# forestagostinelli/DeepCubeA

Hardware: AMD Instinct MI355X
Metric: A* nodes expanded/sec on cube3, batch 20k (higher is better)
Workload: dtype u8 states / f64 cost keys / f32 heuristic

## Files before the change

### deepcubea_amd/csrc/dca_engine.hip

```cpp
#include <string.h>

#include <new>
#include <vector>

#include "dca_common.h"
#include "dca_tile.h"

namespace dca {

constexpr int NBIN = 4096;
constexpr int kBinsPerThread = NBIN / 1024;
constexpr int kLgNbin = 12;
constexpr int kSub = 2048;
constexpr int kScanBlocks = 256;
constexpr int kCollectBlocks = 512;
constexpr int kRankBlocks = 256;
constexpr uint32_t kTinyBin = 512;
constexpr int kSortCap = 8192;
constexpr int RT = 512;
constexpr int kRegEnt = 16;
constexpr uint32_t kLdsEnt = RT * kRegEnt;
constexpr int kStash = 2560;
constexpr int kSegs = NBIN + 1 + kSub;
constexpr uint32_t kGiantBin = 8192;
constexpr int kMaxLevels = 9;
constexpr unsigned long long kBarrierTimeout = 200000000ull;
constexpr unsigned long long kBarrierTimeoutFirst = 25000000ull;
constexpr uint32_t GBAR_BROKEN = 0x80000000u;
constexpr uint32_t NIL = 0xFFFFFFFFu;
constexpr uint32_t ID_MASK = 0x7FFFFFFFu, ID_SOLVED = 0x80000000u;
constexpr uint64_t EMPTY = ~0ull;
constexpr uint64_t DEAD = ~0ull;
constexpr uint32_t GINF = 0xFFFFFFFFu;
constexpr int kMaxMoves = 4096;

struct Slot {
    uint64_t entry;
    uint32_t g;
    uint32_t head;
};

struct alignas(128) Cnt {
    uint32_t v;
    uint32_t pad[31];
};
struct alignas(128) GRange {
    uint64_t kmin, kmax;
    uint32_t imin, imax;
    uint32_t pad[26];
};
struct alignas(128) Rng {
    uint64_t kmin, kmax;
    uint64_t pad[14];
};
struct IterState {
    uint32_t pool_n;
    uint32_t npop, m, base;
    uint32_t best_id;
    int32_t has_best;
    float best_cost;
};
struct Ctl {
    int32_t done, failed, stop_after, pad0;
    int64_t iters, gen, expanded;
    IterState S[2];
    uint32_t cur_f;
    uint32_t hbin;
    uint32_t front_above;
    uint32_t cur_b;
    uint64_t T;
    uint32_t refill, compact, r_bstar, spill_bin, r_move;
    uint64_t r_kmin;
    uint32_t r_shift;
    uint32_t want, bstar, shift, n_big, n_ord;
    uint32_t giant;
    uint32_t tseg;
    uint32_t pre_b, cn_star;
    uint64_t sel_kmin;
    uint32_t goal_id;
    uint32_t dbg_nord, dbg_maxbin, dbg_giant, dbg_giant_seen, dbg_maxsub;
    Cnt open_n[4];
    Cnt closed_n, back_dead, front_dead, ret_n, ticket_a;
    Cnt gbar;
    GRange grange;
    Rng rng[4];
    alignas(128) unsigned long long goal_best;
    alignas(128) uint32_t first_solved;
};

__device__ __forceinline__ uint64_t key_of_cost(double c) {
    uint64_t b = (uint64_t)__double_as_longlong(c);
    return (b & 0x8000000000000000ull) ? ~b : (b | 0x8000000000000000ull);
}
__device__ __forceinline__ double cost_of_key(uint64_t k) {
    uint64_t b = (k & 0x8000000000000000ull) ? (k & 0x7FFFFFFFFFFFFFFFull) : ~k;
    return __longlong_as_double((long long)b);
}
__device__ __forceinline__ uint32_t select_shift(uint64_t kmin, uint64_t kmax) {
    uint64_t range = kmax - kmin;
    int bits = range ? 64 - __clzll((long long)range) : 0;
    return bits > kLgNbin ? (uint32_t)(bits - kLgNbin) : 0u;
}
__device__ __forceinline__ uint32_t bin_of(uint64_t k, uint64_t kmin, uint32_t shift) {
    if (k <= kmin) return 0u;
    const uint64_t f = (k - kmin) >> shift;
    return f < (uint64_t)NBIN ? (uint32_t)f : (uint32_t)(NBIN - 1);
}
__device__ __forceinline__ bool pair_less(uint64_t ka, uint32_t ia, uint64_t kb, uint32_t ib) {
    return ka < kb || (ka == kb && (ia & ID_MASK) < (ib & ID_MASK));
}

enum {
    P_REFILL_HIST = 0, P_REFILL_SCAN, P_REFILL_MOVE, P_SEL_HIST, P_SEL_SCAN, P_SEL_COLLECT, P_RANK, P_EXPAND,
    P_PROBE,
    P_DECIDE, P_PACK, P_COMMIT, P_RANK_SMALL, P_RANK_BIG, P_RB_LOAD, P_RB_COUNT, P_RB_SCATTER, P_RB_ORDER, P_COUNT
};
constexpr int kProfSlots = 1024;
__device__ int g_back_squeeze_mark;
__device__ int g_first_barrier_gives_up;
__device__ __forceinline__ uint32_t rank_shares(uint32_t cn) {
    return cn <= (uint32_t)(512 * 16) ? (cn + 1023u) / 1024u : 1u;
}

struct Eng {
    int env, dim, D, A, B, sem, oh_dtype, depth;
    double w;
    float wf;
    uint32_t max_nodes, M, tab_cap, tab_mask;
    uint32_t front_cap;
    uint8_t* state;
    int32_t* g;
    uint32_t* parent;
    uint8_t* move;
    uint8_t* solved;
    Slot* tab;
    uint32_t* closed_slots;
    uint64_t* open_key[4];
    uint32_t* open_id[4];
    uint32_t f_keep, f_max;
    uint32_t *hist, *pre, *fill;
    uint32_t* rhist;
    uint32_t* subhist;
    int coop;
    uint32_t* coop_off;
    uint64_t* part;
    uint64_t* tmp_key;
    uint32_t* tmp_id;
    uint16_t* tmp_f;
    uint32_t* tmp_idx;
    uint64_t* ord_key;
    uint32_t* ord_id;
    uint32_t* big_list;
    uint64_t* pop_key;
    uint32_t *pop_id, *pop_g;
// ... 660 lines not shown
        s_nbig = 0;
        s_spill = NBIN;
        s_bstar = 0;
        s_hbin = NBIN;
    }
    scan_vals(hv, pre, wsum);
    const uint32_t n = rebased ? (cb ? on1 : on0) : (cb ? on1 : on0) - dead0 - above0;
    const uint32_t want = n < (uint32_t)E.B ? n : (uint32_t)E.B;
    const uint32_t hwant = (uint32_t)(kRefillPeriod + 2) * (uint32_t)E.B;
    for (int k = 0; k < kBinsPerThread; k++) {
        int bin = kBinsPerThread * t + k;
        if (pre[bin] < want && want <= pre[bin + 1]) s_bstar = (uint32_t)bin;
        if (rebased && n > E.f_max) {
            const uint32_t keepn = want + front_keep(E);
            if (pre[bin] < keepn && keepn <= pre[bin + 1]) s_spill = (uint32_t)bin;
        }
        if (rebased && pre[bin] < hwant && hwant <= pre[bin + 1]) s_hbin = (uint32_t)bin + 1u;
        E.pre[bin] = pre[bin];
        E.fill[bin] = 0;
    }
    for (int i = NBIN + t; i < kSegs; i += 1024) E.fill[i] = 0;
    if (t == 1023) E.pre[NBIN] = pre[NBIN];
    __syncthreads();
    const bool giant = E.coop && !*E.coop_off && want != 0 && pre[s_bstar + 1] - pre[s_bstar] > kGiantBin;
    if (giant)
        for (int i = t; i < kMaxLevels * kSub; i += 1024) E.subhist[i] = 0;
    for (int k = 0; k < kBinsPerThread; k++) {
        const uint32_t bin = kBinsPerThread * t + k;
        if (bin <= s_bstar && want != 0) {
            const uint32_t cn = pre[bin + 1] - pre[bin];
            if (cn > 256) atomicMax(&s_maxbin, cn);
            if (cn > (uint32_t)kSortCap) atomicAdd(&s_giant, 1u);
            if (cn > kTinyBin && !(giant && bin == s_bstar)) {
                uint32_t G = rank_shares(cn);
                G = G > 8u ? 8u : G;
                const uint32_t at = atomicAdd(&s_nbig, G);
                for (uint32_t g = 0; g < G; g++) E.big_list[at + g] = bin | (g << 16) | (G << 20);
            }
        }
    }
    __syncthreads();
    if (t == 0) {
        if (rebased) {
            uint64_t fmn = ~0ull, fmx = 0;
            for (int w = 0; w < 16; w++) {
                fmn = s_red[0][w] < fmn ? s_red[0][w] : fmn;
                fmx = s_red[1][w] > fmx ? s_red[1][w] : fmx;
            }
            c->cur_f = cb;
            c->rng[cb].kmin = fmn;
            c->rng[cb].kmax = fmx;
            c->hbin = s_hbin;
        }
        if (refill) {
            if (compact) {
                c->cur_b ^= 1;
                c->back_dead.v = 0;
                c->compact = 0;
            }
            c->refill = 0;
        }
        c->want = want;
        c->bstar = s_bstar;
        c->tseg = s_bstar;
        c->pre_b = pre[s_bstar];
        c->cn_star = pre[s_bstar + 1] - pre[s_bstar];
        c->giant = giant ? 1u : 0u;
        c->gbar.v = 0;
        c->grange.kmin = ~0ull;
        c->grange.kmax = 0;
// ... 259 lines not shown
            subpre[PER * t + k] = run;
            if (run < need && need <= run + v[k]) L.tsub = PER * t + k;
            run += v[k];
        }
        if (t == 255) subpre[kSub] = run;
        __syncthreads();
        tsub = L.tsub;
        if (tsub == ~0u) {
            if (t == 0) c->failed = 1, c->done = 1;
            return BAR_FAIL;
        }
        const uint32_t cn = subpre[tsub + 1] - subpre[tsub];
        if (cn <= kGiantBin || shc == 0 || lvl + 1 >= kMaxLevels) break;
        below += subpre[tsub];
        need -= subpre[tsub];
        V0 += (u128)tsub << shc;
        span = ((u128)1 << shc) - 1;
        __syncthreads();
    }
    const uint32_t seg0 = bstar + 1u;
    if (blockIdx.x == 0) {
        if (t == 0) {
            L.nb = c->n_big;
            E.pre[bstar + 1] = pre_b + below;
            c->tseg = seg0 + tsub;
            c->n_ord = pre_b + below + subpre[tsub + 1];
            c->dbg_nord = pre_b + below + subpre[tsub + 1];
        }
        __syncthreads();
        for (uint32_t sg = t; sg <= tsub + 1u; sg += 256) {
            const uint32_t cn = sg == 0 ? below : subpre[sg] - subpre[sg - 1];
            if (sg > 0) E.pre[seg0 + sg] = pre_b + below + subpre[sg];
            if (cn > kTinyBin) {
                uint32_t G = rank_shares(cn);
                G = G > 8u ? 8u : G;
                const uint32_t at = atomicAdd(&L.nb, G);
                for (uint32_t g = 0; g < G; g++) E.big_list[at + g] = (bstar + sg) | (g << 16) | (G << 20);
            }
        }
        __syncthreads();
        if (t == 0) c->n_big = L.nb;
    }
    uint32_t* lcnt = L.lcnt;
    for (uint32_t i = t; i < (uint32_t)(kSegs + 3); i += 256) lcnt[i] = 0;
    if (t == 0) {
        L.st_n = 0;
        L.nz_n = 0;
    }
    __syncthreads();
    uint64_t* st_key = L.u.g.st_key;
    uint32_t* st_idx = L.u.g.st_idx;
    uint16_t *st_f = L.u.g.st_f, *nzf = L.u.g.nzf;
    auto seg_base = [&](uint32_t f) -> uint32_t {
        return f < bstar ? L.pre[f] : f == bstar ? pre_b : pre_b + below + subpre[f - seg0];
    };
    auto seg_end = [&](uint32_t f) -> uint32_t {
        return f < bstar ? L.pre[f + 1] : f == bstar ? pre_b + below : pre_b + below + subpre[f - seg0 + 1];
    };
    auto flush = [&]() {
        const uint32_t ns = L.st_n < (uint32_t)kStashG ? L.st_n : (uint32_t)kStashG;
        const uint32_t nz = L.nz_n;
        for (uint32_t i = t; i < nz; i += 256) {
            const uint32_t f = nzf[i];
            lcnt[f] = atomicAdd(&E.fill[f], lcnt[f]);
        }
        __syncthreads();
        for (uint32_t p = t; p < ns; p += 256) {
            const uint32_t f = st_f[p];
            const uint32_t id = ids[st_idx[p]];
            const uint32_t pos = seg_base(f) + atomicAdd(&lcnt[f], 1u);
// ... 122 lines not shown
        const uint32_t want = P.want;
#pragma unroll
        for (int k = 0; k < PER; k++) {
            L.pre[PER * t + k] = run;
            if (run < want && want <= run + v[k]) L.bstar = PER * t + k;
            run += v[k];
        }
        if (t == 255) L.pre[NBIN] = run;
        __syncthreads();
        if (want == 0) {
            if (blockIdx.x == 0 && t == 0) {
                c->failed = 1;
                c->done = 1;
            }
            return;
        }
        P.bstar = L.bstar;
        P.pre_b = L.pre[P.bstar];
        P.cn_star = L.pre[P.bstar + 1] - P.pre_b;
        P.giant = E.coop && !*E.coop_off && P.cn_star > kGiantBin;
        if (blockIdx.x == 0) {
            for (uint32_t i = t; i <= (uint32_t)NBIN; i += 256) E.pre[i] = L.pre[i];
            if (t == 0) {
                L.nb = 0;
                L.st_n = 0;
                L.nz_n = 0;
            }
            __syncthreads();
            for (uint32_t bin = t; bin <= P.bstar; bin += 256) {
                const uint32_t cn = L.pre[bin + 1] - L.pre[bin];
                if (cn > 256) atomicMax(&L.st_n, cn);
                if (cn > (uint32_t)kSortCap) atomicAdd(&L.nz_n, 1u);
                if (cn > kTinyBin && !(P.giant && bin == P.bstar)) {
                    uint32_t G = rank_shares(cn);
                    G = G > 8u ? 8u : G;
                    const uint32_t at = atomicAdd(&L.nb, G);
                    for (uint32_t g = 0; g < G; g++) E.big_list[at + g] = bin | (g << 16) | (G << 20);
                }
            }
            __syncthreads();
            if (t == 0) {
                c->bstar = P.bstar;
                c->tseg = P.bstar;
                c->giant = P.giant ? 1u : 0u;
                c->pre_b = P.pre_b;
                c->cn_star = P.cn_star;
                c->spill_bin = NBIN;
                c->n_big = L.nb;
                c->n_ord = L.pre[P.bstar + 1];
                c->front_dead.v += want;
                c->dbg_nord = L.pre[P.bstar + 1];
                c->dbg_maxbin = L.st_n;
                c->dbg_giant = L.nz_n;
                c->dbg_giant_seen += L.nz_n;
                c->dbg_maxsub = 0;
            }
            __syncthreads();
        }
    } else {
        P.bstar = c->bstar;
        P.giant = c->giant != 0;
        P.pre_b = c->pre_b;
        P.cn_star = c->cn_star;
        if (P.want == 0) return;
        for (uint32_t i = t; i <= P.bstar + 1u; i += 256) L.pre[i] = E.pre[i];
        __syncthreads();
    }
    if (P.giant) {
        if (collect_giant(E, c, L, P) != BAR_BROKEN) return;
        if (blockIdx.x == 0 && t == 0) {
            const uint32_t cn = P.cn_star;
            uint32_t G = rank_shares(cn);
            G = G > 8u ? 8u : G;
            const uint32_t at = c->n_big;
            if (cn > kTinyBin) {
                for (uint32_t g = 0; g < G; g++) E.big_list[at + g] = P.bstar | (g << 16) | (G << 20);
                c->n_big = at + G;
            }
            c->giant = 0;
        }
        P.giant = false;
        __syncthreads();
    }
    const uint32_t n = P.n;
    const uint64_t kmin = P.kmin;
    const uint32_t shift = P.shift, bstar = P.bstar;
    uint64_t* __restrict__ keys = E.open_key[P.b];
    const uint32_t* __restrict__ ids = E.open_id[P.b];
    constexpr uint32_t ITEMS = 8, TILE = 256 * ITEMS;
    const uint32_t ntiles = (n + TILE - 1) / TILE;
    uint64_t* st_key = L.u.n.st_key;
    uint32_t* st_idx = L.u.n.st_idx;
    uint16_t *st_f = L.u.n.st_f, *nzf = L.u.n.nzf;
    for (int i = t; i < NBIN; i += 256) L.lcnt[i] = 0;
    if (t == 0) {
        L.st_n = 0;
        L.nz_n = 0;
    }
    __syncthreads();
    auto flush = [&]() {
        const uint32_t ns = L.st_n < (uint32_t)kStash ? L.st_n : (uint32_t)kStash;
        const uint32_t nz = L.nz_n;
        for (uint32_t i = t; i < nz; i += 256) {
            const uint32_t f = nzf[i];
            L.lcnt[f] = atomicAdd(&E.fill[f], L.lcnt[f]);
        }
        __syncthreads();
        for (uint32_t p = t; p < ns; p += 256) {
            const uint32_t f = st_f[p];
// ... 111 lines not shown
    basep = __shfl(basep, leader);
    if (back) {
        const uint32_t slot = E.tmp_idx[basep + (uint32_t)__popcll(mask & ((1ull << lane) - 1ull))];
        E.open_key[nf][slot] = key;
        E.open_id[nf][slot] = id;
    }
}
__device__ __forceinline__ void ret_begin(Ctl* c, RankShared& S, uint32_t nf, uint32_t count) {
    __syncthreads();
    if (threadIdx.x == 0) {
        S.ret_base = count ? atomicAdd(&c->ret_n.v, count) : 0u;
        S.ret_cnt = 0;
    }
    __syncthreads();
}
struct RetAcc {};
__device__ __forceinline__ void ret_put(const Eng& E, Ctl* c, RankShared& S, uint32_t nf, bool pred, uint64_t key,
                                        uint32_t id, RetAcc& acc) {
    const unsigned long long mask = __ballot(pred);
    if (mask == 0) return;
    const int lane = threadIdx.x & 63;
    const int leader = __ffsll((long long)mask) - 1;
    uint32_t basep = 0;
    if (lane == leader) basep = atomicAdd(&S.ret_cnt, (uint32_t)__popcll(mask));
    basep = __shfl(basep, leader);
    if (pred) {
        const uint32_t slot = E.tmp_idx[S.ret_base + basep + (uint32_t)__popcll(mask & ((1ull << lane) - 1ull))];
        E.open_key[nf][slot] = key;
        E.open_id[nf][slot] = id;
    }
}
__device__ __forceinline__ void ret_end(Ctl* c, uint32_t nf, RetAcc acc) {}
template <int NJ>
__device__ __forceinline__ void ret_put_many(const Eng& E, RankShared& S, uint32_t nf, uint32_t n_ord, uint32_t preds,
                                             const uint64_t* key, const uint32_t* id) {
    const uint32_t cnt = (uint32_t)__popc(preds);
    const int lane = threadIdx.x & 63;
    uint32_t incl = cnt;
    for (int o = 1; o < 64; o <<= 1) {
        const uint32_t u = __shfl_up(incl, o);
        if (lane >= o) incl += u;
    }
    const uint32_t total = __shfl(incl, 63);
    if (total == 0) return;
    uint32_t basep = 0;
    if (lane == 63) basep = atomicAdd(&S.ret_cnt, total);
    basep = __shfl(basep, 63);
    uint32_t r = S.ret_base + basep + incl - cnt;
    uint32_t slot[NJ];
#pragma unroll
    for (int j = 0; j < NJ; j++) {
        slot[j] = E.tmp_idx[r < n_ord ? r : n_ord - 1];
        r += (preds >> j) & 1u;
    }
#pragma unroll
    for (int j = 0; j < NJ; j++)
        if ((preds >> j) & 1u) {
            E.open_key[nf][slot[j]] = key[j];
            E.open_id[nf][slot[j]] = id[j];
        }
}

__device__ __forceinline__ void rank_small_entries(const Eng& E, Ctl* c, RankShared& S, uint64_t* LK, uint32_t* LI,
                                                   uint32_t nf, uint32_t p0, uint32_t n_ord, uint32_t want) {
    const uint32_t t = threadIdx.x;
    const uint32_t plast = (p0 + RT - 1 < n_ord ? p0 + RT - 1 : n_ord - 1);
    const uint32_t f_lo = E.tmp_f[p0], f_hi = E.tmp_f[plast];
    const uint32_t lo = E.pre[f_lo], hi = E.pre[f_hi + 1];
    const bool staged = hi - lo <= kLdsEnt && f_hi - f_lo + 2 <= (uint32_t)kSub;
    if (staged) {
        for (uint32_t i = t; i < hi - lo; i += RT) {
            LK[i] = E.tmp_key[lo + i];
            LI[i] = E.tmp_id[lo + i];
        }
        for (uint32_t i = t; i < f_hi - f_lo + 2; i += RT) S.off[i] = E.pre[f_lo + i];
    }
    __syncthreads();
    const uint32_t p = p0 + t;
    bool live = p < n_ord;
    uint64_t k = 0;
    uint32_t id = 0, rank = 0;
    if (live) {
        const uint32_t f = E.tmp_f[p];
        const uint32_t o = staged ? S.off[f - f_lo] : E.pre[f], e = staged ? S.off[f - f_lo + 1] : E.pre[f + 1];
        if (e - o > kTinyBin) {
            live = false;
        } else if (staged) {
            k = LK[p - lo];
            id = LI[p - lo];
            rank = o;
            for (uint32_t j = o - lo; j < e - lo; j++) rank += pair_less(LK[j], LI[j], k, id) ? 1u : 0u;
        } else {
            k = E.tmp_key[p];
            id = E.tmp_id[p];
            rank = o;
            for (uint32_t j = o; j < e; j++) rank += pair_less(E.tmp_key[j], E.tmp_id[j], k, id) ? 1u : 0u;
        }
    }
    emit_ranked(E, c, nf, live, rank, want, k, id);
    __syncthreads();
}

__device__ __forceinline__ uint32_t sub_of(uint64_t k, uint32_t id, u128 vmin, uint32_t shc, uint32_t nsub) {
    const u128 q = (comp_of(k, id) - vmin) >> shc;
    return q < (u128)nsub ? (uint32_t)q : nsub - 1u;
}


__device__ __forceinline__ void rank_range(RankShared& S, u128 vmin, u128 vmax) {
    const uint32_t t = threadIdx.x, lane = t & 63, wv = t >> 6;
    for (int o = 32; o > 0; o >>= 1) {
        uint64_t ahi = __shfl_xor((uint64_t)(vmin >> 64), o), alo = __shfl_xor((uint64_t)vmin, o);
        uint64_t bhi = __shfl_xor((uint64_t)(vmax >> 64), o), blo = __shfl_xor((uint64_t)vmax, o);
        u128 a = ((u128)ahi << 64) | alo, b = ((u128)bhi << 64) | blo;
        vmin = a < vmin ? a : vmin;
        vmax = b > vmax ? b : vmax;
// ... 177 lines not shown
        rank_prefix(S, nsub, need);
        prof_end(E, P_RB_COUNT);
        prof_begin(E, P_RB_SCATTER);
        if (E.prof != nullptr) {
            uint32_t mx = 0;
            for (uint32_t sb = t; sb < nsub; sb += RT) mx = max(mx, S.off[sb + 1] - S.off[sb]);
            if (mx > 16) atomicMax(&c->dbg_maxsub, mx);
        }
        const uint32_t tsub = S.tsub;
        const bool tsub_pushed = S.off[tsub + 1] - S.off[tsub] > kSubMax && refinable;
        const uint32_t in_hi = hi_sub < tsub + 1u ? hi_sub : tsub + 1u;
        const uint32_t ret_lo = lo_sub > tsub + 1u ? lo_sub : tsub + 1u;
        ret_begin(c, S, nf, (ret_lo < hi_sub ? S.off[hi_sub] - S.off[ret_lo] : 0u) +
                                ((tsub >= lo_sub && tsub < hi_sub && !tsub_pushed) ? S.off[tsub + 1] - need : 0u));
        const uint32_t n_ord = c->n_ord;
        {
            uint32_t inm = 0, retm = 0, pos[kRegEnt];
#pragma unroll
            for (int j = 0; j < kRegEnt; j++) {
                const uint32_t sub = (uint32_t)(ek[j] >> shc);
                const bool live = t + (uint32_t)RT * j < n, in = live && sub >= lo_sub && sub < in_hi;
                inm |= (in ? 1u : 0u) << j;
                retm |= (live && sub >= ret_lo && sub < hi_sub ? 1u : 0u) << j;
                pos[j] = S.off[in ? sub : 0u] + atomicAdd(&S.cnt[in ? sub : (uint32_t)kSub + (t & 63u)], in ? 1u : 0u);
            }
#pragma unroll
            for (int j = 0; j < kRegEnt; j++) {
                if ((inm >> j) & 1u) {
                    LK[pos[j]] = ek[j];
                    LI[pos[j]] = ei[j];
                }
                ek[j] = idmode ? kbase : kbase + ek[j];
            }
            ret_put_many<kRegEnt>(E, S, nf, n_ord, retm, ek, ei);
        }
        __syncthreads();
        prof_end(E, P_RB_SCATTER);
        prof_begin(E, P_RB_ORDER);
        const uint32_t p_lo = S.off[lo_sub], p_hi = in_hi > lo_sub ? S.off[in_hi] : p_lo;
        constexpr int U = 4;
        for (uint32_t p0 = p_lo; p0 < p_hi; p0 += RT * U) {
            uint64_t o[U];
            uint32_t id[U], s0[U], cn[U], rank[U], livem = 0, bigm = 0, trip = 0;
#pragma unroll
            for (int u = 0; u < U; u++) {
                const uint32_t p = p0 + (uint32_t)u * RT + t;
                livem |= (p < p_hi ? 1u : 0u) << u;
                o[u] = LK[p < p_hi ? p : p_hi - 1];
                id[u] = LI[p < p_hi ? p : p_hi - 1];
            }
#pragma unroll
            for (int u = 0; u < U; u++) {
                const uint32_t sub = (uint32_t)(o[u] >> shc);
                s0[u] = S.off[sub];
                cn[u] = S.off[sub + 1] - s0[u];
                rank[u] = s0[u];
                if (!((livem >> u) & 1u)) cn[u] = 0;
                if (cn[u] > kSubMax && refinable) {
                    bigm |= 1u << u;
                    cn[u] = 0;
                }
                trip = cn[u] > trip ? cn[u] : trip;
            }
            for (uint32_t jj = 0; jj < trip; jj++) {
#pragma unroll
                for (int u = 0; u < U; u++) {
                    const uint32_t j = s0[u] + (jj < cn[u] ? jj : 0u);
                    const bool less = pair_less(LK[j], LI[j], o[u], id[u]);
                    rank[u] += (jj < cn[u] && less) ? 1u : 0u;
                }
            }
            uint32_t retm = 0;
#pragma unroll
            for (int u = 0; u < U; u++) {
                const uint32_t p = p0 + (uint32_t)u * RT + t;
                o[u] = idmode ? kbase : kbase + o[u];
                if ((bigm >> u) & 1u) {
                    K2[p] = o[u];
                    I2[p] = id[u];
                } else if ((livem >> u) & 1u) {
                    if (rank[u] < need) emit_pop(E, c, it.off + rank[u], o[u], id[u]);
                    else retm |= 1u << u;
                }
            }
            ret_put_many<U>(E, S, nf, n_ord, retm, o, id);
        }
        rank_push(S, it, tsub, need, refinable, lo_sub, in_hi);
        __syncthreads();
        prof_end(E, P_RB_ORDER);
        return;
    }
    {
        u128 vmin = ~(u128)0, vmax = 0;
        for (uint32_t b0 = 0; b0 < n; b0 += kLdsEnt) {
            uint64_t ek[kRegEnt];
            uint32_t ei[kRegEnt];
#pragma unroll
            for (int j = 0; j < kRegEnt; j++) {
                const uint32_t i = b0 + t + (uint32_t)RT * j, ic = i < n ? i : n - 1;
                ek[j] = K[ic];
                ei[j] = I[ic];
            }
#pragma unroll
            for (int j = 0; j < kRegEnt; j++)
                if (b0 + t + (uint32_t)RT * j < n) {
                    const u128 v = comp_of(ek[j], ei[j]);
                    vmin = v < vmin ? v : vmin;
                    vmax = v > vmax ? v : vmax;
                }
        }
        rank_range(S, vmin, vmax);
    }
    const u128 base = ((u128)S.vmin_hi << 64) | S.vmin_lo;
    const uint32_t bits = S.bits;
    if (lg > bits) lg = bits;
    const uint32_t nsub = 1u << lg, shc = bits - lg;
    for (uint32_t b0 = 0; b0 < n; b0 += kLdsEnt) {
        uint64_t ek[kRegEnt];
// ... 9 lines not shown
            if (b0 + t + (uint32_t)RT * j < n) atomicAdd(&S.cnt[sub_of(ek[j], ei[j], base, shc, nsub)], 1u);
    }
    __syncthreads();
    rank_prefix(S, nsub, need);
    const uint32_t tsub = S.tsub;
    const bool tsub_pushed = S.off[tsub + 1] - S.off[tsub] > kSubMax && shc > 0;
    ret_begin(c, S, nf, (n - S.off[tsub + 1]) + (tsub_pushed ? 0u : S.off[tsub + 1] - need));
    RetAcc acc{};
    const uint32_t n_ord_all = c->n_ord;
    for (uint32_t b0 = 0; b0 < n; b0 += kLdsEnt) {
        uint64_t ek[kRegEnt];
        uint32_t ei[kRegEnt];
#pragma unroll
        for (int j = 0; j < kRegEnt; j++) {
            const uint32_t i = b0 + t + (uint32_t)RT * j, ic = i < n ? i : n - 1;
            ek[j] = K[ic];
            ei[j] = I[ic];
        }
        uint32_t retm = 0;
#pragma unroll
        for (int j = 0; j < kRegEnt; j++) {
            const bool live = b0 + t + (uint32_t)RT * j < n;
            uint32_t sub = 0;
            if (live) {
                sub = sub_of(ek[j], ei[j], base, shc, nsub);
                if (sub <= tsub) {
                    const uint32_t p = S.off[sub] + atomicAdd(&S.cnt[sub], 1u);
                    K2[p] = ek[j];
                    I2[p] = ei[j];
                }
            }
            retm |= (live && sub > tsub ? 1u : 0u) << j;
        }
        ret_put_many<kRegEnt>(E, S, nf, n_ord_all, retm, ek, ei);
    }
    __syncthreads();
    const uint32_t m = S.off[tsub + 1];
    for (uint32_t p0 = 0; p0 < m; p0 += RT) {
        const uint32_t p = p0 + t;
        bool live = p < m;
        uint64_t k = 0;
        uint32_t id = 0, rank = 0;
        if (live) {
            k = K2[p];
            id = I2[p];
            const uint32_t sub = sub_of(k, id, base, shc, nsub);
            const uint32_t s0 = S.off[sub], e0 = S.off[sub + 1];
            if (e0 - s0 > kSubMax && shc > 0) {
                live = false;
            } else {
                rank = s0;
                for (uint32_t j = s0; j < e0; j++) rank += pair_less(K2[j], I2[j], k, id) ? 1u : 0u;
                if (rank < need) emit_pop(E, c, it.off + rank, k, id);
            }
        }
        ret_put(E, c, S, nf, live && rank >= need, k, id, acc);
    }
    rank_push(S, it, tsub, need, shc > 0);
    ret_end(c, nf, acc);
    __syncthreads();
}

__global__ __launch_bounds__(RT) void k_rank(const Eng* __restrict__ engs) {
    const Eng& E = engs[blockIdx.y];
    Ctl* c = E.ctl;
    if (c->done) return;
    Stamp stamp(E, P_RANK);
    __shared__ RankShared S;
    extern __shared__ __attribute__((aligned(16))) uint8_t rank_lds[];
    uint64_t* LK = reinterpret_cast<uint64_t*>(rank_lds);
    uint32_t* LI = reinterpret_cast<uint32_t*>(rank_lds + (size_t)kLdsEnt * 8);
    const uint32_t t = threadIdx.x;
    const uint32_t nf = c->cur_f;
    const uint32_t tseg = c->tseg, want = c->want;
    const uint32_t n_big = c->n_big, n_ord = c->n_ord;
    if (blockIdx.x == gridDim.x - 1) {
        const uint32_t bstar = c->bstar, pre_b = c->pre_b, cn_star = c->cn_star;
        if (want != 0) {
            for (uint32_t bin = t; bin < bstar; bin += RT) E.hist[bin] = 0;
            if (t == 0) E.hist[bstar] = cn_star - (want - pre_b);
        }
        for (uint32_t i = t; i < (uint32_t)kSegs; i += RT) E.fill[i] = 0;
        if (c->giant)
            for (uint32_t i = t; i < (uint32_t)(kMaxLevels * kSub); i += RT) E.subhist[i] = 0;
    }
    {
        Stamp sub(E, P_RANK_SMALL);
        for (uint32_t p0 = blockIdx.x * RT; p0 < n_ord; p0 += gridDim.x * RT)
            rank_small_entries(E, c, S, LK, LI, nf, p0, n_ord, want);
    }
    Stamp sub2(E, P_RANK_BIG);
    for (uint32_t bi = (blockIdx.x + gridDim.x - 64u) % gridDim.x; bi < n_big; bi += gridDim.x) {
        const uint32_t unit = E.big_list[bi];
        const uint32_t f = unit & 0xFFFFu;
        const uint32_t o = E.pre[f], n = E.pre[f + 1] - o;
        __syncthreads();
        if (t == 0) {
            S.stack[0] = RankItem{o, n, (f == tseg) ? want - o : n, 0u, (unit >> 16) & 15u, unit >> 20, 0u};
            S.sp = 1;
            S.fail = 0;
        }
        for (;;) {
            __syncthreads();
            const uint32_t sp = S.sp;
            if (sp == 0 || sp > (uint32_t)kRankStack) break;
            const RankItem it = S.stack[sp - 1];
            __syncthreads();
            if (t == 0) S.sp = sp - 1;
            __syncthreads();
            rank_item(E, c, S, LK, LI, nf, want, it);
        }
        if (t == 0 && (S.fail || S.sp != 0)) c->failed = 1;
    }
}

__device__ __forceinline__ void close_pop(const Eng& E, Ctl* c, const IterState& S0, uint32_t it, uint32_t want,
                                          uint32_t npop, uint32_t base, bool fail) {
    IterState N = S0;
    if (E.sem == DCA_SEM_PY) {
        const unsigned long long gb = c->goal_best;
        if (gb != ~0ull) {
            c->stop_after = 1;
            c->goal_id = E.pop_id[(uint32_t)(gb & 0xFFFFFFFFull)] & ID_MASK;
        }
    } else {
        const uint32_t fs = c->first_solved;
        if (fs != NIL) {
            const float cst = (float)cost_of_key(E.pop_key[fs]);
            if (E.B == 1) {
                N.best_id = E.pop_id[fs] & ID_MASK;
                N.best_cost = cst;
// ... 1065 lines not shown
        E.f_max = 3 * E.f_keep;
        E.tab_cap = (uint32_t)cap;
        E.tab_mask = (uint32_t)(cap - 1);
        E.nnet_in = e->nnet_all + i * M * D;
        E.child_h = e->h_all + i * M;
        E.onehot = e->onehot_all ? e->onehot_all + i * M * D * depth * (onehot_dtype == DCA_DT_F32 ? 4 : 2) : nullptr;
#define ALLOC(field, count) \
    if (!rc) rc = dev_alloc(e, &E.field, (count))
        ALLOC(state, N * D + 64);
        ALLOC(g, N);
        ALLOC(parent, N);
        ALLOC(move, N);
        ALLOC(solved, N);
        ALLOC(tab, (size_t)cap);
        ALLOC(closed_slots, N);
        ALLOC(coop_off, 16);
        E.front_cap = (uint32_t)(N + (size_t)(2 * kRefillPeriod) * Bz);
        for (int b = 0; b < 4; b++) {
            ALLOC(open_key[b], b < 2 ? (size_t)E.front_cap : N);
            ALLOC(open_id[b], b < 2 ? (size_t)E.front_cap : N);
        }
        ALLOC(hist, NBIN);
        ALLOC(rhist, NBIN);
        ALLOC(pre, kSegs + 16);
        ALLOC(fill, kSegs + 8);
        ALLOC(subhist, (size_t)kMaxLevels * kSub);
        ALLOC(part, 4 * 1024);
        ALLOC(tmp_key, N);
        ALLOC(tmp_id, N);
        ALLOC(tmp_f, N);
        ALLOC(tmp_idx, N);
        ALLOC(ord_key, N);
        ALLOC(ord_id, N);
        ALLOC(big_list, 8 * kSegs);
        ALLOC(pop_key, Bz);
        ALLOC(pop_id, Bz);
        ALLOC(pop_g, Bz);
        ALLOC(child_slot, M);
        ALLOC(child_next, M);
        ALLOC(child_flags, M);
        ALLOC(child_v0, M);
        ALLOC(child_multi, M);
        ALLOC(root_nnet, 64);
        ALLOC(d_moves, kMaxMoves);
        ALLOC(ctl, 1);
#undef ALLOC
        if (!rc) {
            (void)hipMemset(E.hist, 0, NBIN * sizeof(uint32_t));
            (void)hipMemset(E.rhist, 0, NBIN * sizeof(uint32_t));
            (void)hipMemset(E.fill, 0, (kSegs + 8) * sizeof(uint32_t));
            (void)hipMemset(E.subhist, 0, (size_t)kMaxLevels * kSub * sizeof(uint32_t));
            (void)hipMemset(E.child_multi, 0, M);
            (void)hipMemset(E.coop_off, 0, 16 * sizeof(uint32_t));
            (void)hipMemset(E.ctl, 0, sizeof(Ctl));
        }
    }
    if (!rc) {
        hipError_t err = hipHostMalloc((void**)&e->h_ctl, sizeof(Ctl) + kMaxMoves * sizeof(int32_t) + 512);
        if (err != hipSuccess) rc = hip_fail(err, "hipHostMalloc");
    }
    if (!rc) {
        hipError_t err = hipFuncSetAttribute(reinterpret_cast<const void*>(k_sel_collect<false>),
                                             hipFuncAttributeMaxDynamicSharedMemorySize, (int)sizeof(CollectLds));
        if (err == hipSuccess)
            err = hipFuncSetAttribute(reinterpret_cast<const void*>(k_sel_collect<true>),
                                      hipFuncAttributeMaxDynamicSharedMemorySize, (int)sizeof(CollectLds));
        if (err != hipSuccess) rc = hip_fail(err, "hipFuncSetAttribute(k_sel_collect)");
// ... 522 lines not shown
    return 0;
}
int dca_engine_status(dca_engine* e, dca_status* out, void* stream) {
    return dca_engine_status_instance(e, 0, out, stream);
}

int dca_engine_debug(dca_engine* e, double* out, void* stream) {
    DCA_ARG(e != nullptr && out != nullptr);
    if (int rc = fetch_ctl(e, 0, (hipStream_t)stream)) return rc;
    const Ctl& c = *e->h_ctl;
    auto cost = [](uint64_t k) {
        uint64_t b = (k & 0x8000000000000000ull) ? (k & 0x7FFFFFFFFFFFFFFFull) : ~k;
        double d;
        memcpy(&d, &b, 8);
        return d;
    };
    const IterState& S = c.S[(c.iters + (e->phase != 0 ? 1 : 0)) & 1];
    out[0] = (double)c.open_n[c.cur_f].v - (double)c.front_dead.v;
    out[1] = (double)c.open_n[c.cur_b].v - (double)c.back_dead.v;
    out[2] = cost(c.rng[c.cur_f].kmin);
    out[3] = cost(c.rng[c.cur_f].kmax);
    out[4] = cost(c.rng[c.cur_b].kmin);
    out[5] = cost(c.rng[c.cur_b].kmax);
    out[6] = cost(c.T);
    out[7] = c.want;
    out[8] = c.bstar;
    out[9] = c.dbg_nord;
    out[10] = c.dbg_maxbin;
    out[11] = c.dbg_giant_seen;
    out[12] = c.dbg_maxsub;
    out[13] = c.spill_bin;
    out[14] = S.npop;
    out[15] = S.m;
    return 0;
}

int dca_engine_last_children(dca_engine* e, const uint8_t** states, int64_t* m_live, void* stream) {
    DCA_ARG(e != nullptr && states != nullptr && m_live != nullptr);
    if (int rc = fetch_ctl(e, 0, (hipStream_t)stream)) return rc;
    const IterState& S = e->h_ctl->S[(e->h_ctl->iters + (e->phase != 0 ? 1 : 0)) & 1];
    *states = e->E[0].state + (size_t)S.base * e->E[0].D;
    *m_live = S.m;
    return 0;
}

int dca_engine_solution_instance(dca_engine* e, int inst, int32_t* moves, int cap, int* len, double* path_cost,
                                 void* stream) {
    DCA_INST(e, inst);
    DCA_ARG(len != nullptr && cap >= 0 && (cap == 0 || moves != nullptr));
    hipStream_t s = (hipStream_t)stream;
    const Eng& E = e->E[inst];
    hipLaunchKernelGGL(k_solution, dim3(1), dim3(64), 0, s, E, E.d_moves, e->d_cost);
    if (int rc = launch_check("k_solution")) return rc;
    DCA_HIP(hipMemcpyAsync(e->h_moves, E.d_moves, kMaxMoves * sizeof(int32_t), hipMemcpyDeviceToHost, s));
    DCA_HIP(hipMemcpyAsync(e->h_cost, e->d_cost, sizeof(double), hipMemcpyDeviceToHost, s));
    DCA_HIP(hipStreamSynchronize(s));
    int n = e->h_moves[0];
    if (n < 0) {
        set_error("no solution recorded (search not finished)");
        return DCA_E_NOTFOUND;
    }
    *len = n;
    if (path_cost) *path_cost = *e->h_cost;
    for (int i = 0; i < n && i < cap; i++) moves[i] = e->h_moves[1 + i];
    return 0;
}
// ... 5 lines not shown
```

### deepcubea_amd/search_methods/engine.py

```python
from __future__ import annotations

import ctypes as C
from typing import Callable, List, Optional, Tuple

import numpy as np
import torch

from .. import _lib

_OH = {None: -1, torch.float32: _lib.DT_F32, torch.float16: _lib.DT_F16, torch.bfloat16: _lib.DT_BF16}


class BwasEngine:

    def __init__(self, env_name: str, weight: float, batch_size: int, max_nodes: int = 1 << 24,
                 semantics: int = _lib.SEM_PY, onehot_dtype: Optional[torch.dtype] = None, num_instances: int = 1,
                 packed: bool = False, onehot_stride: Optional[int] = None):
        _lib.require_gpu()
        self.env_id, self.dim, self.state_dim, self.num_moves, self.depth = _lib.env_ids(env_name)
        self.batch_size = int(batch_size)
        self.weight = float(weight)
        self.semantics = semantics
        self.onehot_dtype = onehot_dtype
        self.num_instances = int(num_instances)
# ... 148 lines not shown
            except AttributeError:
                pass
            h = heuristic_fn_dev(oh[:n], True) if oh is not None else heuristic_fn_dev(nn[:n])
            assert h.shape[0] >= rows
            self.commit_packed(h.to(torch.float32).contiguous())
            return
        self.rows_evaluated += self.m_capacity
        nn, oh = self.pop_expand()
        h = heuristic_fn_dev(oh, True) if oh is not None else heuristic_fn_dev(nn)
        self.commit(h.to(torch.float32).contiguous())

    def run_builtin(self, heur_id: int, iters: int, use_graph: bool = False) -> None:
        _lib.check(_lib.lib().dca_engine_run_builtin(self._h, heur_id, int(iters), int(use_graph),
                                                     _lib.stream_ptr()), "dca_engine_run_builtin")

    PROF_SLOTS = ["refill_hist", "refill_scan", "refill_move", "sel_hist", "sel_scan", "sel_collect", "rank", "expand",
                  "probe", "decide", "pack", "commit", "rank_small", "rank_big", "rank_big_load", "rank_big_count",
                  "rank_big_scatter", "rank_big_order"]

    def profile_builtin(self, heur_id: int, iters: int, use_graph: bool = True) -> dict:
        n = len(self.PROF_SLOTS)
        span, gap = (C.c_float * n)(), (C.c_float * n)()
        _lib.check(_lib.lib().dca_engine_profile_builtin(self._h, heur_id, int(iters), int(use_graph), span, gap,
                                                         _lib.stream_ptr()), "dca_engine_profile_builtin")
        it = max(iters, 1)
        return {"span_ms": {nm: span[k] / it for k, nm in enumerate(self.PROF_SLOTS) if span[k] > 0},
                "gap_ms": {nm: gap[k] / it for k, nm in enumerate(self.PROF_SLOTS) if span[k] > 0}}

    def set_tiers(self, front_keep: int, front_max: int) -> None:
        _lib.check(_lib.lib().dca_engine_set_tiers(self._h, C.c_int64(front_keep), C.c_int64(front_max)),
                   "dca_engine_set_tiers")

    def debug(self) -> dict:
        out = (C.c_double * 16)()
        _lib.check(_lib.lib().dca_engine_debug(self._h, out, _lib.stream_ptr()), "dca_engine_debug")
        names = ["front_n", "back_n", "front_cmin", "front_cmax", "back_cmin", "back_cmax", "T", "want", "bstar",
                 "n_ord", "max_bin", "giant_bins_seen", "max_sub", "spill_bin", "npop", "m"]
        return dict(zip(names, list(out)))

    def status(self, instance: int = 0) -> dict:
        st = _lib.DcaStatus()
        _lib.check(_lib.lib().dca_engine_status_instance(self._h, int(instance), C.byref(st), _lib.stream_ptr()),
                   "dca_engine_status_instance")
        return {k: getattr(st, k) for k, _ in _lib.DcaStatus._fields_}

    def last_children(self) -> torch.Tensor:
        p, m = C.c_void_p(0), C.c_int64(0)
        _lib.check(_lib.lib().dca_engine_last_children(self._h, C.byref(p), C.byref(m), _lib.stream_ptr()),
                   "dca_engine_last_children")
        return _wrap_u8(p.value, (m.value, self.state_dim))

    def solution(self, instance: int = 0) -> Tuple[List[int], float]:
        moves = np.zeros(4096, np.int32)
        n, pc = C.c_int(0), C.c_double(0)
        _lib.check(_lib.lib().dca_engine_solution_instance(self._h, int(instance), moves.ctypes.data_as(C.c_void_p),
                                                           moves.size, C.byref(n), C.byref(pc), _lib.stream_ptr()),
                   "dca_engine_solution_instance")
        return moves[:n.value].tolist(), float(pc.value)

    def solve_builtin(self, root: np.ndarray, heur_id: int, max_iters: int = 1 << 30, chunk: int = 16,
                      use_graph: bool = False) -> dict:
        self.reset(root)
        if self.semantics == _lib.SEM_PY:
            h0 = _lib.heuristic_builtin(heur_id, torch.from_numpy(np.ascontiguousarray(root, np.uint8)[None]).cuda())
            self.root_commit(h0)
        it = 0
        while it < max_iters:
            n = min(chunk, max_iters - it)
            self.run_builtin(heur_id, n, use_graph)
            it += n
# ... 86 lines not shown
```

Measured before the change: 94.69 million.

## Rank mid-sized bins by all-pairs counting instead of radix bucketing

Adds an all-pairs rank path for big bins of up to 4096 entries. Each bin is staged into shared memory, and groups of 8 lanes count how many entries precede each element. Entries are spread over several shares per bin, and big-list units now carry the bin offset and size. The small-bin threshold is lowered to 256, so more bins take the big-bin path, and new debug counters record pairs/bucket bin statistics each rank pass. The change replaces iterative sub-histogram ranking with O(n^2) comparisons that parallelise well. In exchange it costs more ALU work per bin, a larger big_list allocation, and extra per-iteration counting and atomics in block 0.

```diff
diff --git a/deepcubea_amd/csrc/dca_engine.hip b/deepcubea_amd/csrc/dca_engine.hip
--- a/deepcubea_amd/csrc/dca_engine.hip
+++ b/deepcubea_amd/csrc/dca_engine.hip
@@ -15,11 +15,17 @@
 constexpr int kScanBlocks = 256;
 constexpr int kCollectBlocks = 512;
 constexpr int kRankBlocks = 256;
-constexpr uint32_t kTinyBin = 512;
+constexpr uint32_t kTinyBin = 256;
 constexpr int kSortCap = 8192;
 constexpr int RT = 512;
 constexpr int kRegEnt = 16;
 constexpr uint32_t kLdsEnt = RT * kRegEnt;
+constexpr uint32_t kAllPairsMax = 4096;
+constexpr int kPairLanes = 8;
+constexpr int kPairRegs = 4;
+constexpr uint32_t kPairEnt = RT / kPairLanes * kPairRegs;
+constexpr uint32_t kMaxShares = (kAllPairsMax + kPairEnt - 1) / kPairEnt;
+static_assert(kAllPairsMax <= kLdsEnt && kAllPairsMax % RT == 0 && kMaxShares >= 8 && kMaxShares < 256, "unit encoding / staging");
 constexpr int kStash = 2560;
 constexpr int kSegs = NBIN + 1 + kSub;
 constexpr uint32_t kGiantBin = 8192;
@@ -79,6 +85,7 @@
     uint64_t sel_kmin;
     uint32_t goal_id;
     uint32_t dbg_nord, dbg_maxbin, dbg_giant, dbg_giant_seen, dbg_maxsub;
+    uint32_t dbg_pairs, dbg_pairs_min, dbg_pairs_max, dbg_bucket;
     Cnt open_n[4];
     Cnt closed_n, back_dead, front_dead, ret_n, ticket_a;
     Cnt gbar;
@@ -119,7 +126,11 @@
 __device__ int g_back_squeeze_mark;
 __device__ int g_first_barrier_gives_up;
 __device__ __forceinline__ uint32_t rank_shares(uint32_t cn) {
-    return cn <= (uint32_t)(512 * 16) ? (cn + 1023u) / 1024u : 1u;
+    if (cn <= kAllPairsMax) return (cn + kPairEnt - 1u) / kPairEnt;
+    return cn <= kLdsEnt ? (cn + 1023u) / 1024u : 1u;
+}
+__device__ __forceinline__ void rank_list_units(uint32_t* list, uint32_t at, uint32_t seg, uint32_t G, uint32_t o, uint32_t n) {
+    for (uint32_t g = 0; g < G; g++) reinterpret_cast<uint4*>(list)[at + g] = make_uint4(seg | (g << 16) | (G << 24), o, n, 0u);
 }
 
 struct Eng {
@@ -846,10 +857,8 @@
             if (cn > 256) atomicMax(&s_maxbin, cn);
             if (cn > (uint32_t)kSortCap) atomicAdd(&s_giant, 1u);
             if (cn > kTinyBin && !(giant && bin == s_bstar)) {
-                uint32_t G = rank_shares(cn);
-                G = G > 8u ? 8u : G;
-                const uint32_t at = atomicAdd(&s_nbig, G);
-                for (uint32_t g = 0; g < G; g++) E.big_list[at + g] = bin | (g << 16) | (G << 20);
+                const uint32_t G = rank_shares(cn);
+                rank_list_units(E.big_list, atomicAdd(&s_nbig, G), bin, G, pre[bin], cn);
             }
         }
     }
@@ -1175,10 +1184,8 @@
             const uint32_t cn = sg == 0 ? below : subpre[sg] - subpre[sg - 1];
             if (sg > 0) E.pre[seg0 + sg] = pre_b + below + subpre[sg];
             if (cn > kTinyBin) {
-                uint32_t G = rank_shares(cn);
-                G = G > 8u ? 8u : G;
-                const uint32_t at = atomicAdd(&L.nb, G);
-                for (uint32_t g = 0; g < G; g++) E.big_list[at + g] = (bstar + sg) | (g << 16) | (G << 20);
+                const uint32_t G = rank_shares(cn);
+                rank_list_units(E.big_list, atomicAdd(&L.nb, G), bstar + sg, G, sg == 0 ? pre_b : pre_b + below + subpre[sg] - cn, cn);
             }
         }
         __syncthreads();
@@ -1367,10 +1374,8 @@
                 if (cn > 256) atomicMax(&L.st_n, cn);
                 if (cn > (uint32_t)kSortCap) atomicAdd(&L.nz_n, 1u);
                 if (cn > kTinyBin && !(P.giant && bin == P.bstar)) {
-                    uint32_t G = rank_shares(cn);
-                    G = G > 8u ? 8u : G;
-                    const uint32_t at = atomicAdd(&L.nb, G);
-                    for (uint32_t g = 0; g < G; g++) E.big_list[at + g] = bin | (g << 16) | (G << 20);
+                    const uint32_t G = rank_shares(cn);
+                    rank_list_units(E.big_list, atomicAdd(&L.nb, G), bin, G, L.pre[bin], cn);
                 }
             }
             __syncthreads();
@@ -1405,11 +1410,10 @@
         if (collect_giant(E, c, L, P) != BAR_BROKEN) return;
         if (blockIdx.x == 0 && t == 0) {
             const uint32_t cn = P.cn_star;
-            uint32_t G = rank_shares(cn);
-            G = G > 8u ? 8u : G;
+            const uint32_t G = rank_shares(cn);
             const uint32_t at = c->n_big;
             if (cn > kTinyBin) {
-                for (uint32_t g = 0; g < G; g++) E.big_list[at + g] = P.bstar | (g << 16) | (G << 20);
+                rank_list_units(E.big_list, at, P.bstar, G, P.pre_b, cn);
                 c->n_big = at + G;
             }
             c->giant = 0;
@@ -1587,8 +1591,8 @@
 }
 __device__ __forceinline__ void ret_end(Ctl* c, uint32_t nf, RetAcc acc) {}
 template <int NJ>
-__device__ __forceinline__ void ret_put_many(const Eng& E, RankShared& S, uint32_t nf, uint32_t n_ord, uint32_t preds,
-                                             const uint64_t* key, const uint32_t* id) {
+__device__ __forceinline__ void ret_put_many(const Eng& E, uint32_t* counter, uint32_t base, uint32_t nf, uint32_t n_ord,
+                                             uint32_t preds, const uint64_t* key, const uint32_t* id) {
     const uint32_t cnt = (uint32_t)__popc(preds);
     const int lane = threadIdx.x & 63;
     uint32_t incl = cnt;
@@ -1599,9 +1603,9 @@
     const uint32_t total = __shfl(incl, 63);
     if (total == 0) return;
     uint32_t basep = 0;
-    if (lane == 63) basep = atomicAdd(&S.ret_cnt, total);
+    if (lane == 63) basep = atomicAdd(counter, total);
     basep = __shfl(basep, 63);
-    uint32_t r = S.ret_base + basep + incl - cnt;
+    uint32_t r = base + basep + incl - cnt;
     uint32_t slot[NJ];
 #pragma unroll
     for (int j = 0; j < NJ; j++) {
@@ -1621,6 +1625,7 @@
     const uint32_t t = threadIdx.x;
     const uint32_t plast = (p0 + RT - 1 < n_ord ? p0 + RT - 1 : n_ord - 1);
     const uint32_t f_lo = E.tmp_f[p0], f_hi = E.tmp_f[plast];
+    const uint32_t f = E.tmp_f[p0 + t < n_ord ? p0 + t : plast];
     const uint32_t lo = E.pre[f_lo], hi = E.pre[f_hi + 1];
     const bool staged = hi - lo <= kLdsEnt && f_hi - f_lo + 2 <= (uint32_t)kSub;
     if (staged) {
@@ -1636,7 +1641,6 @@
     uint64_t k = 0;
     uint32_t id = 0, rank = 0;
     if (live) {
-        const uint32_t f = E.tmp_f[p];
         const uint32_t o = staged ? S.off[f - f_lo] : E.pre[f], e = staged ? S.off[f - f_lo + 1] : E.pre[f + 1];
         if (e - o > kTinyBin) {
             live = false;
@@ -1880,7 +1884,7 @@
                 }
                 ek[j] = idmode ? kbase : kbase + ek[j];
             }
-            ret_put_many<kRegEnt>(E, S, nf, n_ord, retm, ek, ei);
+            ret_put_many<kRegEnt>(E, &S.ret_cnt, S.ret_base, nf, n_ord, retm, ek, ei);
         }
         __syncthreads();
         prof_end(E, P_RB_SCATTER);
@@ -1931,7 +1935,7 @@
                     else retm |= 1u << u;
                 }
             }
-            ret_put_many<U>(E, S, nf, n_ord, retm, o, id);
+            ret_put_many<U>(E, &S.ret_cnt, S.ret_base, nf, n_ord, retm, o, id);
         }
         rank_push(S, it, tsub, need, refinable, lo_sub, in_hi);
         __syncthreads();
@@ -2007,7 +2011,7 @@
             }
             retm |= (live && sub > tsub ? 1u : 0u) << j;
         }
-        ret_put_many<kRegEnt>(E, S, nf, n_ord_all, retm, ek, ei);
+        ret_put_many<kRegEnt>(E, &S.ret_cnt, S.ret_base, nf, n_ord_all, retm, ek, ei);
     }
     __syncthreads();
     const uint32_t m = S.off[tsub + 1];
@@ -2034,6 +2038,58 @@
     rank_push(S, it, tsub, need, shc > 0);
     ret_end(c, nf, acc);
     __syncthreads();
+}
+
+__device__ __forceinline__ void rank_pairs_share(const Eng& E, Ctl* c, uint64_t* LK, uint32_t* LI, uint32_t nf, uint32_t o,
+                                                 uint32_t n, uint32_t g, uint32_t want, uint32_t n_ord) {
+    constexpr int PER = kAllPairsMax / RT;
+    const uint32_t t = threadIdx.x;
+    {
+        uint64_t sk[PER];
+        uint32_t si[PER];
+#pragma unroll
+        for (int j = 0; j < PER; j++) {
+            const uint32_t i = t + (uint32_t)RT * j, ic = i < n ? i : n - 1;
+            sk[j] = E.tmp_key[o + ic];
+            si[j] = E.tmp_id[o + ic];
+        }
+#pragma unroll
+        for (int j = 0; j < PER; j++) {
+            const uint32_t i = t + (uint32_t)RT * j;
+            if (i < n) {
+                LK[i] = sk[j];
+                LI[i] = si[j];
+            }
+        }
+    }
+    __syncthreads();
+    const uint32_t l = t & (uint32_t)(kPairLanes - 1), e0 = g * kPairEnt + t / (uint32_t)kPairLanes;
+    uint64_t k[kPairRegs];
+    uint32_t id[kPairRegs], cnt[kPairRegs];
+#pragma unroll
+    for (int r = 0; r < kPairRegs; r++) {
+        const uint32_t e = e0 + (uint32_t)r * (RT / kPairLanes);
+        k[r] = LK[e < n ? e : n - 1];
+        id[r] = LI[e < n ? e : n - 1];
+        cnt[r] = 0;
+    }
+#pragma unroll 2
+    for (uint32_t j = l; j < n; j += (uint32_t)kPairLanes) {
+        const uint64_t kj = LK[j];
+        const uint32_t ij = LI[j];
+#pragma unroll
+        for (int r = 0; r < kPairRegs; r++) cnt[r] += pair_less(kj, ij, k[r], id[r]) ? 1u : 0u;
+    }
+    uint32_t backm = 0;
+#pragma unroll
+    for (int r = 0; r < kPairRegs; r++) {
+#pragma unroll
+        for (int x = kPairLanes / 2; x > 0; x >>= 1) cnt[r] += __shfl_xor(cnt[r], x);
+        const bool live = l == 0 && e0 + (uint32_t)r * (RT / kPairLanes) < n;
+        if (live && o + cnt[r] < want) emit_pop(E, c, o + cnt[r], k[r], id[r]);
+        backm |= (live && o + cnt[r] >= want ? 1u : 0u) << r;
+    }
+    ret_put_many<kPairRegs>(E, &c->ret_n.v, 0u, nf, n_ord, backm, k, id);
 }
 
 __global__ __launch_bounds__(RT) void k_rank(const Eng* __restrict__ engs) {
@@ -2058,6 +2114,45 @@
         for (uint32_t i = t; i < (uint32_t)kSegs; i += RT) E.fill[i] = 0;
         if (c->giant)
             for (uint32_t i = t; i < (uint32_t)(kMaxLevels * kSub); i += RT) E.subhist[i] = 0;
+        uint32_t np = 0, nb = 0, mn = ~0u, mx = 0;
+        for (uint32_t bi = t; bi < n_big; bi += RT) {
+            const uint4 unit = reinterpret_cast<const uint4*>(E.big_list)[bi];
+            if ((unit.x >> 16) & 0xFFu) continue;
+            const uint32_t n = unit.z;
+            if (n <= kAllPairsMax) {
+                np++;
+                mn = n < mn ? n : mn;
+                mx = n > mx ? n : mx;
+            } else {
+                nb++;
+            }
+        }
+        for (int x = 32; x > 0; x >>= 1) {
+            np += __shfl_xor(np, x);
+            nb += __shfl_xor(nb, x);
+            mn = min(mn, (uint32_t)__shfl_xor(mn, x));
+            mx = max(mx, (uint32_t)__shfl_xor(mx, x));
+        }
+        if ((t & 63u) == 0) {
+            S.cnt[4 * (t >> 6)] = np;
+            S.cnt[4 * (t >> 6) + 1] = nb;
+            S.cnt[4 * (t >> 6) + 2] = mn;
+            S.cnt[4 * (t >> 6) + 3] = mx;
+        }
+        __syncthreads();
+        if (t == 0) {
+            for (int w = 1; w < RT / 64; w++) {
+                np += S.cnt[4 * w];
+                nb += S.cnt[4 * w + 1];
+                mn = min(mn, S.cnt[4 * w + 2]);
+                mx = max(mx, S.cnt[4 * w + 3]);
+            }
+            c->dbg_pairs += np;
+            c->dbg_bucket += nb;
+            if (np && (c->dbg_pairs_min == 0 || mn < c->dbg_pairs_min)) c->dbg_pairs_min = mn;
+            if (mx > c->dbg_pairs_max) c->dbg_pairs_max = mx;
+        }
+        __syncthreads();
     }
     {
         Stamp sub(E, P_RANK_SMALL);
@@ -2065,13 +2160,17 @@
             rank_small_entries(E, c, S, LK, LI, nf, p0, n_ord, want);
     }
     Stamp sub2(E, P_RANK_BIG);
-    for (uint32_t bi = (blockIdx.x + gridDim.x - 64u) % gridDim.x; bi < n_big; bi += gridDim.x) {
-        const uint32_t unit = E.big_list[bi];
-        const uint32_t f = unit & 0xFFFFu;
-        const uint32_t o = E.pre[f], n = E.pre[f + 1] - o;
+    const uint32_t first = min((n_ord + (uint32_t)RT - 1u) / (uint32_t)RT, gridDim.x);
+    for (uint32_t bi = (blockIdx.x + gridDim.x - first) % gridDim.x; bi < n_big; bi += gridDim.x) {
+        const uint4 u4 = reinterpret_cast<const uint4*>(E.big_list)[bi];
+        const uint32_t unit = u4.x, f = unit & 0xFFFFu, o = u4.y, n = u4.z;
         __syncthreads();
+        if (n <= kAllPairsMax) {
+            rank_pairs_share(E, c, LK, LI, nf, o, n, (unit >> 16) & 0xFFu, want, n_ord);
+            continue;
+        }
         if (t == 0) {
-            S.stack[0] = RankItem{o, n, (f == tseg) ? want - o : n, 0u, (unit >> 16) & 15u, unit >> 20, 0u};
+            S.stack[0] = RankItem{o, n, (f == tseg) ? want - o : n, 0u, (unit >> 16) & 0xFFu, unit >> 24, 0u};
             S.sp = 1;
             S.fail = 0;
         }
@@ -3203,7 +3302,7 @@
         ALLOC(tmp_idx, N);
         ALLOC(ord_key, N);
         ALLOC(ord_id, N);
-        ALLOC(big_list, 8 * kSegs);
+        ALLOC(big_list, 4 * kMaxShares * kSegs);
         ALLOC(pop_key, Bz);
         ALLOC(pop_id, Bz);
         ALLOC(pop_g, Bz);
@@ -3792,6 +3891,10 @@
     out[13] = c.spill_bin;
     out[14] = S.npop;
     out[15] = S.m;
+    out[16] = c.dbg_pairs;
+    out[17] = c.dbg_pairs_min;
+    out[18] = c.dbg_pairs_max;
+    out[19] = c.dbg_bucket;
     return 0;
 }
 
diff --git a/deepcubea_amd/search_methods/engine.py b/deepcubea_amd/search_methods/engine.py
--- a/deepcubea_amd/search_methods/engine.py
+++ b/deepcubea_amd/search_methods/engine.py
@@ -204,10 +204,11 @@
                    "dca_engine_set_tiers")
 
     def debug(self) -> dict:
-        out = (C.c_double * 16)()
+        out = (C.c_double * 20)()
         _lib.check(_lib.lib().dca_engine_debug(self._h, out, _lib.stream_ptr()), "dca_engine_debug")
         names = ["front_n", "back_n", "front_cmin", "front_cmax", "back_cmin", "back_cmax", "T", "want", "bstar",
-                 "n_ord", "max_bin", "giant_bins_seen", "max_sub", "spill_bin", "npop", "m"]
+                 "n_ord", "max_bin", "giant_bins_seen", "max_sub", "spill_bin", "npop", "m",
+                 "pairs_bins", "pairs_min", "pairs_max", "bucket_bins"]
         return dict(zip(names, list(out)))
 
     def status(self, instance: int = 0) -> dict:
```

After: 93.49 million. -1.3%, worse.
